# G-U-N/consolver

Hardware: AMD Instinct MI355X
Metric: images/sec at 8-step ConsistencySolver 512x512 (final latents; SD1.5 UNet fp16 + PPOScheduler, CFG 3) (higher is better)
Workload: dtype f16

## Files before the change

consolver_amd/csrc/attention.hip:

```cpp
#include "ops.h"
#include "el.h"
#include <type_traits>


namespace {

struct AttnParams {
    const f16* q; const f16* k; const f16* v; f16* out;
    int q_stride, k_stride, v_stride, out_stride;
    int H, Nq, Nk;
    float c;
    const float* bias;
    int nqb, lin0;
    int splits, tiles_per_split, part_rows;
    float* part_o;
    float* part_ml;
    int prio;
};

typedef __fp16 hf4 __attribute__((__vector_size__(4 * sizeof(__fp16))));
typedef __attribute__((address_space(3))) hf4* lds_hf4_ptr;

__device__ __forceinline__ u32x2 tr_read(const char* lds_addr) {
    hf4 r = __builtin_amdgcn_ds_read_tr16_b64_v4f16((lds_hf4_ptr)lds_addr);
// ... 758 lines not shown
                    for (int t = 0; t < 4; ++t) {
                        const u32x4 f = {pack2<f16>(s2[2 * t2][t][0], s2[2 * t2][t][1]), pack2<f16>(s2[2 * t2][t][2], s2[2 * t2][t][3]),
                                         pack2<f16>(s2[2 * t2 + 1][t][0], s2[2 * t2 + 1][t][1]), pack2<f16>(s2[2 * t2 + 1][t][2], s2[2 * t2 + 1][t][3])};
                        o_acc[a][t] = El<f16>::mfma(as_frag<f16>(vv.v), as_frag<f16>(f), o_acc[a][t]);
                    }
                }
            }
        }
#pragma unroll
        for (int t = 0; t < 4; ++t) lsum[t] = __shfl(o_acc[2][t][0], 32 + i16, 64);
    }
#pragma unroll
    for (int t = 0; t < 4; ++t) {
        const float inv = 1.0f / lsum[t];
        const int qrow = q0 + t * 16 + i16;
        f16* orow = p.out + (size_t)(b * p.Nq + qrow) * p.out_stride + h * DH;
#pragma unroll
        for (int a = 0; a < 3; ++a) {
            const int d = a * 16 + 4 * g;
            if (d + 4 <= DH) {
                const u32x2 o = {pack2<f16>(o_acc[a][t][0] * inv, o_acc[a][t][1] * inv), pack2<f16>(o_acc[a][t][2] * inv, o_acc[a][t][3] * inv)};
                *reinterpret_cast<u32x2*>(orow + d) = o;
            }
        }
    }
    if (TRACE && w == 0 && lane == 0 && blockIdx.x < A40_TRACE_SLOTS) {
        unsigned long long* tr = g_a40_trace + blockIdx.x * A40_TRACE_W;
        const unsigned long long te4 = __builtin_amdgcn_s_memrealtime();
        tr[5] = te1 - te0; tr[6] = tr0 - te1; tr[7] = te4 - te3; tr[8] = te0; tr[9] = te4;
        tr[10] = ((unsigned long long)__builtin_amdgcn_s_getreg((4 - 1) << 11 | 0 << 6 | 20) << 32) | __builtin_amdgcn_s_getreg((32 - 1) << 11 | 0 << 6 | 4);
    }
}

constexpr int ATTN_SLOTS = 512;

template <typename T, int DH, int QT, bool CAUSAL = false, bool BIAS = false>
int launch_attn(AttnParams p, int B, hipStream_t s, void* split_ws = nullptr, size_t split_ws_bytes = 0) {
    constexpr int DK = (DH + 31) / 32 * 32, DVP = (DH + 15) / 16 * 16;
    constexpr int KS = (DK == 64) ? 128 : ((DK * 2) % 64 == 32 ? DK * 2 : DK * 2 + 32);
    constexpr int VS = ((DVP * 2) % 64 == 32) ? DVP * 2 : DVP * 2 + 32;
    constexpr size_t lds = 2 * 64 * (size_t)(KS + VS);
    auto kfn = attn_kernel<T, DH, QT, CAUSAL, BIAS>;
    static bool configured = false;
    if (!configured) {
        CS_CHECK_HIP(hipFuncSetAttribute(reinterpret_cast<const void*>(kfn), hipFuncAttributeMaxDynamicSharedMemorySize, (int)lds));
        configured = true;
    }
    constexpr int ROWS = 4 * QT * 16;
    p.nqb = (p.Nq + ROWS - 1) / ROWS; p.lin0 = 0; p.splits = 1; p.tiles_per_split = 0; p.part_rows = 0; p.part_o = nullptr; p.part_ml = nullptr;
    const long total = (long)p.nqb * p.H * B;
    if (total > 0x7fffffffL) CS_FAIL(CS_E_SHAPE, "attention: too many workgroups");
    long main_wgs = total;
    if constexpr (DH == 128 && !CAUSAL && !BIAS) {
        const long tail = total % ATTN_SLOTS;
        const int tiles = (p.Nk + 63) / 64;
        if (split_ws && total > ATTN_SLOTS && tail > 0 && tail * 2 <= ATTN_SLOTS && tiles >= 8) {
            int splits = (int)std::min<long>(std::min<long>(ATTN_SLOTS / tail, 8), tiles / 4);
            const int per = (tiles + splits - 1) / splits;
            splits = (tiles + per - 1) / per;
            const size_t rows = (size_t)tail * ROWS;
            const size_t need = (size_t)splits * rows * (DH + 2) * sizeof(float);
            if (splits >= 2 && need <= split_ws_bytes) {
                main_wgs = total - tail;
                hipLaunchKernelGGL(kfn, dim3((unsigned)main_wgs), dim3(256), lds, s, p);
                AttnParams t = p;
                t.lin0 = (int)main_wgs; t.splits = splits; t.tiles_per_split = per; t.part_rows = (int)rows;
// ... 9 lines not shown
                CS_CHECK_LAUNCH();
                return CS_OK;
            }
        }
    }
    hipLaunchKernelGGL(kfn, dim3((unsigned)main_wgs), dim3(256), lds, s, p);
    CS_CHECK_LAUNCH();
    return CS_OK;
}

constexpr int A40_NS = 6;
int launch_attn40_lw(AttnParams p, int B, hipStream_t s) {
    constexpr size_t lds = (size_t)A40_NS * 12288;
    const bool trace = (tune().debug & 16384) != 0;
    auto kfn = trace ? ((tune().debug & 1) ? attn40_lw_kernel<A40_NS, true, 1> : (tune().debug & 2) ? attn40_lw_kernel<A40_NS, true, 2> : attn40_lw_kernel<A40_NS, true>)
                     : tune().attn_lw == 2 ? attn40_lw_kernel<A40_NS, false, 0, 0, false> : attn40_lw_kernel<A40_NS, false>;
    static bool configured = false;
    if (!configured) {
        CS_CHECK_HIP(hipFuncSetAttribute(reinterpret_cast<const void*>(attn40_lw_kernel<A40_NS, false>), hipFuncAttributeMaxDynamicSharedMemorySize, (int)lds));
        CS_CHECK_HIP(hipFuncSetAttribute(reinterpret_cast<const void*>(attn40_lw_kernel<A40_NS, false, 0, 0, false>), hipFuncAttributeMaxDynamicSharedMemorySize, (int)lds));
        CS_CHECK_HIP(hipFuncSetAttribute(reinterpret_cast<const void*>(attn40_lw_kernel<A40_NS, true>), hipFuncAttributeMaxDynamicSharedMemorySize, (int)lds));
        CS_CHECK_HIP(hipFuncSetAttribute(reinterpret_cast<const void*>(attn40_lw_kernel<A40_NS, true, 1>), hipFuncAttributeMaxDynamicSharedMemorySize, (int)lds));
        CS_CHECK_HIP(hipFuncSetAttribute(reinterpret_cast<const void*>(attn40_lw_kernel<A40_NS, true, 2>), hipFuncAttributeMaxDynamicSharedMemorySize, (int)lds));
        configured = true;
    }
    p.nqb = p.Nq / 256; p.lin0 = 0; p.splits = 1; p.tiles_per_split = 0; p.part_rows = 0; p.part_o = nullptr; p.part_ml = nullptr;
    const long total = (long)p.nqb * p.H * B;
    if (total > 0x7fffffffL) CS_FAIL(CS_E_SHAPE, "attention: too many workgroups");
    hipLaunchKernelGGL(kfn, dim3((unsigned)total), dim3(512), lds, s, p);
    CS_CHECK_LAUNCH();
    return CS_OK;
}

}

int debug_attn_trace_read(void* dst, size_t bytes) {
    if (bytes > sizeof(unsigned long long) * A40_TRACE_SLOTS * A40_TRACE_W) bytes = sizeof(unsigned long long) * A40_TRACE_SLOTS * A40_TRACE_W;
    return hipMemcpyFromSymbol(dst, HIP_SYMBOL(g_a40_trace), bytes, 0, hipMemcpyDeviceToHost) == hipSuccess ? CS_OK : CS_E_HIP;
}

size_t attention_split_workspace_bytes(int B, int H, int Nq, int Nk, int dh) {
    if (dh != 128) return 0;
    const long total = (long)((Nq + 127) / 128) * H * B, tail = total % ATTN_SLOTS;
    if (total <= ATTN_SLOTS || tail == 0 || tail * 2 > ATTN_SLOTS || (Nk + 63) / 64 < 8) return 0;
    return (size_t)8 * tail * 128 * (dh + 2) * sizeof(float);
}

int launch_attention(const AttnArgs& a, hipStream_t s) {
    if (!a.q || !a.k || !a.v || !a.out) CS_FAIL(CS_E_ARG, "attention: null pointer");
    if (a.B <= 0 || a.Nq <= 0) return a.B < 0 ? CS_E_SHAPE : CS_OK;
    if (a.Nk <= 0) CS_FAIL(CS_E_SHAPE, "attention: Nk must be positive");
    if ((a.q_stride | a.k_stride | a.v_stride | a.out_stride) & 7) CS_FAIL(CS_E_SHAPE, "attention: strides must be multiples of 8 halfs");
    AttnParams p;
    p.q = a.q; p.k = a.k; p.v = a.v; p.out = a.out;
    p.q_stride = a.q_stride; p.k_stride = a.k_stride; p.v_stride = a.v_stride; p.out_stride = a.out_stride;
    p.H = a.H; p.Nq = a.Nq; p.Nk = a.Nk;
    p.c = a.scale * 1.4426950408889634f;
    p.bias = a.bias;
    p.prio = tune().attn_prio < 0 ? (a.dh == 128 ? 1 : 0) : tune().attn_prio;
    if (a.bias) {
        if (a.dh != 64 || a.causal || a.Nk % 4) CS_FAIL(CS_E_UNSUPPORTED, "attention: the biased form is built for head dim 64, no mask, Nk %% 4 == 0");
        if (a.dtype == CS_BF16) return launch_attn<bf16_el, 64, 2, false, true>(p, a.B, s);
        return launch_attn<f16, 64, 2, false, true>(p, a.B, s);
    }
    if (a.causal) {
        if (a.dh != 64 || a.dtype == CS_BF16 || a.Nq != a.Nk) CS_FAIL(CS_E_UNSUPPORTED, "attention: the causal form is built for f16, head dim 64, Nq == Nk");
        return launch_attn<f16, 64, 2, true>(p, a.B, s);
    }
    switch (a.dh) {
        case 40: {
            const int qt = tune().attn_qt40;
            if (a.dtype == CS_BF16) CS_FAIL(CS_E_UNSUPPORTED, "attention: bf16 is built for head dim 128 only");
            if (tune().attn_lw && qt == 4 && a.Nq % 256 == 0 && a.Nk % 64 == 0) return launch_attn40_lw(p, a.B, s);
            if (qt == 4) return launch_attn<f16, 40, 4>(p, a.B, s);
            return launch_attn<f16, 40, 2>(p, a.B, s);
        }
        case 80: if (a.dtype == CS_BF16) break; return launch_attn<f16, 80, 2>(p, a.B, s);
        case 160: if (a.dtype == CS_BF16) break; return launch_attn<f16, 160, 1>(p, a.B, s);
        case 128:
            if (a.dtype == CS_BF16) return launch_attn<bf16_el, 128, 2>(p, a.B, s, a.split_ws, a.split_ws_bytes);
            return launch_attn<f16, 128, 2>(p, a.B, s, a.split_ws, a.split_ws_bytes);
        default: break;
    }
    CS_FAIL(CS_E_UNSUPPORTED, "attention: head dim %d / dtype %d not built (f16: 40/80/160/128, bf16: 128)", a.dh, a.dtype);
}
```

consolver_amd/csrc/ops.h:

```cpp
#pragma once
#include "common.h"

struct TuneSet {
    int halo = 1;
    int conv_lw = 1;
    int gemm_w8 = 1;
    int gemm_lw = 1;
    int gemm2_w8 = 1;
    int attn_lw = 1;
    int debug = 0;
    int gemm_gm = -1;
    int gn_fuse = 1;
    int cfg_share = 1;
    int xattn_fused = 1;
    int attn_prio = -1;
    int gemm2_prio = 0;
    int biggemm = 1;
    int attn_qt40 = 4;
    int x2_split_a = 1;
    int x2_sc_skip = 0;
    int ln_fold = 1;
    int xcd_grid = 1;
    int epi_fast = 3;
    int lo8 = 1;
    int conv_in_mfma = 1;
    int up_fold = 1;
    int head_x2 = 1;
    int conv_out_mfma = 1;
    int xattn_tile = 64;
};
extern TuneSet g_tune;
extern thread_local const TuneSet* t_tune;
inline const TuneSet& tune() { return t_tune ? *t_tune : g_tune; }
struct TuneScope {
    const TuneSet* prev;
    explicit TuneScope(const TuneSet* t) : prev(t_tune) { t_tune = t; }
    ~TuneScope() { t_tune = prev; }
    TuneScope(const TuneScope&) = delete; TuneScope& operator=(const TuneScope&) = delete;
};
int tune_apply(TuneSet& set, const char* key, int value);
TuneSet tune_snapshot();

// ... 131 lines not shown
```

consolver_amd/csrc/ops_api.cpp:

```cpp
#include "ops.h"
#include "../../include/consolver_hip_ops.h"
#include <cstring>

int debug_trace_read(void* dst, size_t bytes);
int debug_attn_trace_read(void* dst, size_t bytes);

#include <mutex>
TuneSet g_tune;
thread_local const TuneSet* t_tune = nullptr;
static std::mutex g_tune_write_mutex;

struct TuneKnob { const char* key; int TuneSet::* var; int lo, hi; bool pair; };
static const TuneKnob* tune_knobs(int* n) {
    static const TuneKnob k[] = {
        {"conv_halo", &TuneSet::halo, 0, 4, false},     {"gemm_lw", &TuneSet::gemm_lw, 0, 1, false},      {"gemm2_w8", &TuneSet::gemm2_w8, 0, 1, false},
        {"attn_lw", &TuneSet::attn_lw, 0, 2, false},    {"gemm_w8", &TuneSet::gemm_w8, 0, 1, false},      {"conv_lw", &TuneSet::conv_lw, 0, 3, false},
        {"gemm_big", &TuneSet::biggemm, 0, 3, false},   {"debug", &TuneSet::debug, 0, 0x7fffffff, false}, {"gemm_gm", &TuneSet::gemm_gm, -1, 64, false},
        {"gn_fuse", &TuneSet::gn_fuse, 0, 1, false},    {"xattn_fused", &TuneSet::xattn_fused, 0, 1, false}, {"cfg_share", &TuneSet::cfg_share, 0, 1, false},
        {"gemm2_prio", &TuneSet::gemm2_prio, -1, 1, false}, {"attn_prio", &TuneSet::attn_prio, -1, 1, false}, {"attn_qt40", &TuneSet::attn_qt40, 2, 4, true},
        {"x2_split_a", &TuneSet::x2_split_a, 0, 3, false}, {"x2_sc_skip", &TuneSet::x2_sc_skip, 0, 0xffff, false}, {"ln_fold", &TuneSet::ln_fold, 0, 1, false}, {"xcd_grid", &TuneSet::xcd_grid, 0, 1, false}, {"epi_fast", &TuneSet::epi_fast, 0, 3, false}, {"lo8", &TuneSet::lo8, 0, 1, false},
        {"conv_in_mfma", &TuneSet::conv_in_mfma, 0, 1, false}, {"xattn_tile", &TuneSet::xattn_tile, 64, 128, true},
        {"conv_out_mfma", &TuneSet::conv_out_mfma, 0, 1, false},
        {"up_fold", &TuneSet::up_fold, 0, 2, false},
        {"head_x2", &TuneSet::head_x2, 0, 1, false},
    };
    *n = (int)(sizeof(k) / sizeof(k[0]));
    return k;
}

int tune_apply(TuneSet& set, const char* key, int value) {
    if (!key) CS_FAIL(CS_E_ARG, "key is NULL");
    int n; const TuneKnob* k = tune_knobs(&n);
    for (int i = 0; i < n; ++i)
        if (!strcmp(key, k[i].key)) {
            const bool ok = k[i].pair ? (value == k[i].lo || value == k[i].hi) : (value >= k[i].lo && value <= k[i].hi);
            if (!ok) CS_FAIL(CS_E_ARG, "tuning key '%s': value %d outside %s%d%s%d%s", key, value, k[i].pair ? "{" : "[", k[i].lo, k[i].pair ? ", " : " .. ", k[i].hi, k[i].pair ? "}" : "]");
            set.*(k[i].var) = value;
            return CS_OK;
        }
    CS_FAIL(CS_E_ARG, "unknown tuning key '%s'", key);
}

TuneSet tune_snapshot() {
    std::lock_guard<std::mutex> lock(g_tune_write_mutex);
    return g_tune;
}

extern "C" {

int cs_set_tuning(const char* key, int value) {
    std::lock_guard<std::mutex> lock(g_tune_write_mutex);
    return tune_apply(g_tune, key, value);
}

int cs_get_tuning(const char* key, int* value) {
    if (!key || !value) CS_FAIL(CS_E_ARG, "key / value is NULL");
    int n; const TuneKnob* k = tune_knobs(&n);
// ... 321 lines not shown
```

consolver_amd/csrc/igemm.hip:

```cpp
#include "ops.h"
#include <stdlib.h>
#include <type_traits>


namespace {

constexpr int BM = 128;
constexpr int BK = 64;

__device__ __attribute__((aligned(256))) unsigned g_zero_page[64];

struct IgemmParams {
    const f16* a0; const f16* a1; int c0, c1;
    int Hi, Wi, Ho, Wo, HoWo;
    int stride, upsample;
    int pad_lo;
    int M, N, KT, cpt;
    int Ktot;
    const f16* w; const f16* bias; const f16* temb; int temb_stride; const f16* res; f16* out;
    const f16* res_lo; f16* out_lo;
    const f16* a0_lo; const f16* a1_lo; int KTh;
    float* row_stats;
    const float* ln_stats; int ln_groups; float ln_inv_c, ln_eps; const float* ln_s; const float* ln_b;
    int tiles_n, nblk;
// ... 1063 lines not shown
        g_trace[blockIdx.x * CS_TRACE_W + 5] = (unsigned long long)nsteps;
        g_trace[blockIdx.x * CS_TRACE_W + 0] = tw_entry;
        g_trace[blockIdx.x * CS_TRACE_W + 1] = tc_r0;
        g_trace[blockIdx.x * CS_TRACE_W + 2] = __builtin_amdgcn_s_memrealtime();
        g_trace[blockIdx.x * CS_TRACE_W + 4] = ((unsigned long long)__builtin_amdgcn_s_getreg((4 - 1) << 11 | 0 << 6 | 20) << 32) | __builtin_amdgcn_s_getreg((32 - 1) << 11 | 0 << 6 | 4);
    }
    __builtin_amdgcn_s_barrier();
    if (btab) __builtin_amdgcn_s_barrier();
    if constexpr (SUB) {
        const SubRows rows{wm * 64, b0, y0, x0, p.B, p.Ho, p.Wo, p.tw_shift, p.trw_shift, phase >> 1, phase & 1, phase * ((p.Ho * p.Wo) >> 8)};
        igemm_epilogue<false, NT, MT, NT, SubRows, 2, 0, true>(p.e, acc, rows, n_blk, lane, smem + w * 11264, btab ? smem + 4 * 11264 : nullptr);
        return;
    }
    const PatchRows rows{wm * 64, b0, y0, x0, p.B, p.Ho, p.Wo, p.tw_shift, p.trw_shift};
    if (p.splits == 1) {
        igemm_epilogue<false, NT, MT, NT, PatchRows, 2, 0, true>(p.e, acc, rows, n_blk, lane, smem + w * 11264, btab ? smem + 4 * 11264 : nullptr);
    } else {
        float* dst = p.partial + (size_t)blockIdx.y * p.e.M * p.e.N;
#pragma unroll
        for (int j = 0; j < MT; ++j) {
            const int m = rows(j * 16 + (lane & 15));
            if (m < 0) continue;
#pragma unroll
            for (int i = 0; i < NT; ++i)
                *reinterpret_cast<f32x4*>(dst + (size_t)m * p.e.N + n_blk + i * 16 + gq * 4) = acc[i][j];
        }
    }
    if (TRACE && w == 0 && lane == 0 && blockIdx.x < CS_TRACE_SLOTS && blockIdx.y == 0) {
        asm volatile("s_waitcnt vmcnt(0)" ::: "memory");
        g_trace[blockIdx.x * CS_TRACE_W + 3] = __builtin_amdgcn_s_memrealtime();
    }
}

template <int LNM = 0, int EPI = 0>
__global__ __launch_bounds__(512, 2) void gemm_lw_kernel(IgemmParams p) {
    constexpr int BMX = 256, BN = 160, NT = BN / 16, MT = 4, NWB = 3;
    constexpr int A_BYTES = BMX * 128, B_BYTES = BN * 128, STAGE = A_BYTES + B_BYTES;
    constexpr int APL = BMX / 8 / 4, WPL = BN / 8 / 4;
    extern __shared__ __attribute__((aligned(16))) char smem[];

    const int tid = threadIdx.x, lane = tid & 63;
    const int w = __builtin_amdgcn_readfirstlane(tid >> 6);
    int tm, tn;
    tile_of(blockIdx.x, p.nblk, p.tiles_n, p.gm, p.pn, tm, tn);
    const int m_blk = tm * BMX, n_blk = tn * BN;
    const int KT = p.KT;
    char* const lnx = smem + NWB * STAGE;

    if (w >= 4) {
        const int l = w - 4;

        const int pch = lane & 7, lr = lane >> 3;
        const f16* asrc0[APL]; const f16* asrc1[APL]; const f16* wsrc[WPL];
#pragma unroll
        for (int j = 0; j < APL; ++j) {
            const int r = 8 * (l + 4 * j) + lr;
            const long m = min(m_blk + r, p.M - 1);
            const int ch = (pch ^ ((r >> 1) & 7)) * 8;
            asrc0[j] = p.a0 + m * p.c0 + ch;
            asrc1[j] = p.c1 ? p.a1 + m * p.c1 + ch : asrc0[j];
        }
#pragma unroll
        for (int j = 0; j < WPL; ++j) {
            const int r = 8 * (l + 4 * j) + lr;
            wsrc[j] = p.w + (size_t)(n_blk + r) * p.Ktot + (pch ^ ((r >> 1) & 7)) * 8;
        }
// ... 660 lines not shown
constexpr size_t LN_LDS_W8 = 256 * 8 + 2 * 2 * 160 * 4, LN_LDS_LW = 256 * 8 + 2 * 160 * 4;

static int choose_xcd_grid(int tiles_m, int tiles_n, double a_bytes, double w_bytes) {
    if (!tune().xcd_grid) return 0;
    int best = 0; double best_cost = 0.85 * (a_bytes + 8.0 * w_bytes);
    for (int pn = 2; pn <= 8; pn *= 2) {
        const int px = 8 / pn;
        if (tiles_n % pn || tiles_m % px) continue;
        const double cost = pn * a_bytes + px * w_bytes;
        if (cost < best_cost) { best_cost = cost; best = pn; }
    }
    return best;
}

double igemm_flops(const IgemmArgs& a) {
    const double M = (double)a.B * a.Ho * a.Wo;
    return 2.0 * M * a.N * (double)a.taps * (a.c0 + a.c1);
}

template <bool UP, int BN, int KH, int SCHED>
static int launch_halo_sched(const HaloParams& h, dim3 grid, size_t lds, hipStream_t s) {
    static bool configured = false;
    if (!configured) {
        constexpr size_t max_lds = 2 * (HALO_ROWS_MAX * 128) + 3 * (160 * 128);
        CS_CHECK_HIP(hipFuncSetAttribute(reinterpret_cast<const void*>(conv3_halo_kernel<UP, BN, KH, SCHED>), hipFuncAttributeMaxDynamicSharedMemorySize, (int)max_lds));
        configured = true;
    }
    hipLaunchKernelGGL((conv3_halo_kernel<UP, BN, KH, SCHED>), grid, dim3(512), lds, s, h);
    CS_CHECK_LAUNCH();
    return CS_OK;
}
template <bool UP, int BN, int KH>
static int launch_halo(const HaloParams& h, dim3 grid, size_t lds, hipStream_t s) { return launch_halo_sched<UP, BN, KH, KH == 2 ? 2 : 0>(h, grid, lds, s); }

struct LaunchInfo { bool gn_done = false; int row_groups = 0; };
static int launch_igemm_impl(const IgemmArgs& a, hipStream_t s, LaunchInfo* li) {
    const int cin = a.c0 + a.c1;
    if (!a.a0 || !a.w || !a.out) CS_FAIL(CS_E_ARG, "igemm: a0, w, out required");
    if (a.taps != 1 && a.taps != 9) CS_FAIL(CS_E_ARG, "igemm: taps must be 1 or 9");
    if (cin % BK || a.c0 % BK || (a.c1 && !a.a1)) CS_FAIL(CS_E_SHAPE, "igemm: channels (%d,%d) must be multiples of %d", a.c0, a.c1, BK);
    if (a.B <= 0 || a.Ho <= 0 || a.Wo <= 0) return (a.B < 0) ? CS_E_SHAPE : CS_OK;
    if (a.taps == 1 && (a.stride != 1 || a.upsample || a.Hi != a.Ho || a.Wi != a.Wo)) CS_FAIL(CS_E_ARG, "igemm: 1x1 needs stride 1, no upsample");
    if (a.geglu && (a.N % 256) && (a.N % 320)) CS_FAIL(CS_E_SHAPE, "igemm: GEGLU needs N %% 256 == 0 or N %% 320 == 0 (N=%d)", a.N);
    IgemmParams p;
    p.a0 = a.a0; p.a1 = a.a1; p.c0 = a.c0; p.c1 = a.c1;
    p.Hi = a.Hi; p.Wi = a.Wi; p.Ho = a.Ho; p.Wo = a.Wo; p.HoWo = a.Ho * a.Wo;
    p.stride = a.stride; p.upsample = a.upsample; p.pad_lo = a.pad_after_only ? 0 : 1;
    if (a.pad_after_only && !(a.taps == 9 && a.stride == 2)) CS_FAIL(CS_E_ARG, "igemm: pad_after_only is the stride-2 3x3 form");
    p.M = a.B * a.Ho * a.Wo; p.N = a.N; p.cpt = cin / BK; p.KT = a.taps * p.cpt; p.Ktot = a.taps * cin;
    p.w = a.w; p.bias = a.bias; p.temb = a.temb; p.temb_stride = a.temb_stride; p.res = a.res; p.out = a.out;
    p.res_lo = a.res ? a.res_lo : nullptr; p.out_lo = a.out_lo; p.lo8 = (a.lo8 && (p.res_lo || p.out_lo)) ? 1 : 0;
    const bool conv3_early = a.taps == 9;
    p.row_stats = a.row_stats;
    p.ln_stats = a.ln_stats; p.ln_groups = a.ln_groups; p.ln_inv_c = 1.0f / (float)cin; p.ln_eps = a.ln_eps; p.ln_s = a.ln_s; p.ln_b = a.ln_b;
    if (a.ln_stats) {
        if (a.taps != 1 || a.c1 || a.temb || a.res || a.out_lo || a.row_stats || a.gn_stats)
            CS_FAIL(CS_E_ARG, "igemm: a folded LayerNorm (ln_stats) is the epilogue of a plain linear layer (one source, no temb / residual / lo plane / statistics)");
        if (!a.ln_s || !a.ln_b || a.ln_groups < 1) CS_FAIL(CS_E_ARG, "igemm: ln_stats needs ln_s, ln_b and ln_groups >= 1");
    }
    if (a.row_stats && (a.geglu || a.gn_stats)) CS_FAIL(CS_E_ARG, "igemm: row_stats excludes GEGLU and gn_stats");
    if (a.row_stats && !a.row_stats_groups) CS_FAIL(CS_E_ARG, "igemm: row_stats needs row_stats_groups (the layout the chosen kernel wrote is returned there)");
    p.a0_lo = a.a0_lo; p.a1_lo = a.c1 ? a.a1_lo : nullptr; p.KTh = p.KT;
    const int lnm = a.ln_stats ? 1 : (a.row_stats && !conv3_early ? 2 : 0);
    const bool split_a = a.a0_lo != nullptr;
    if (split_a) {
        if (a.taps != 1 || a.geglu) CS_FAIL(CS_E_ARG, "igemm: a split-fp16 A operand (a0_lo) is built for 1x1 / linear layers without GEGLU");
// ... 69 lines not shown
        }
        const bool pays = tiles_m * tiles_n * splits >= 160;
        const int tin_w = a.upsample ? TW / 2 : TW, tin_h = a.upsample ? TH / 2 : TH;
        HaloParams h;
        h.HALO_W = tin_w + 2; h.HALO_IMG = (tin_h + 2) * (tin_w + 2); h.NHALO = IPT * h.HALO_IMG; h.NQ = (h.NHALO + 7) / 8;
        if ((pays || use_halo == 2 || use_halo == 3) && h.NHALO <= HALO_ROWS_MAX && h.NQ <= 64 && (PP == 1 || IPT == 1)) {
            h.e = p; h.e.tiles_n = tiles_n; h.e.nblk = tiles_m * tiles_n; h.e.row_stats = nullptr; h.e.pn = choose_xcd_grid(tiles_m, tiles_n, a_bytes, w_bytes);
            h.x = a.a0; h.w = a.w; h.Cin = cin; h.H = a.Hi; h.W = a.Wi; h.B = a.B; h.NC = NC; h.Ho = Ho; h.Wo = Wo;
            h.tw_shift = TW == 16 ? 4 : 3; h.trw_shift = 0; while ((1 << h.trw_shift) < TRW) ++h.trw_shift;
            h.PX = PX; h.PP = PP;
            h.splits = splits; h.partial = a.splitk_ws; h.sched = wide ? 2 : 0;
            const size_t l = 2 * (HALO_ROWS_MAX * 128) + 3 * ((size_t)hbn * (wide ? 64 : 128));
            const dim3 grid(h.e.nblk, splits);
            int rc;
            if (lw) {
                constexpr size_t llw_max = 2 * (HALO_ROWS_MAX * 128) + 3 * (160 * 128);
                const size_t llw = 2 * ((size_t)h.NQ * 1024) + 3 * ((size_t)hbn * 128);
                const bool fast = TW == 16 && TH == 16 && tune().conv_lw != 2 && (a.upsample ? (h.HALO_W == 10 && h.NQ == 13) : (h.HALO_W == 18 && h.NQ == 41));
                const bool fast8 = hbn == 160 && TW == 8 && TH == 8 && !a.upsample && IPT == 4 && PP == 1 && h.HALO_W == 10 && h.NQ == 50 && tune().conv_lw != 2 &&
                                   !((tune().debug & 16384) != 0);
                typedef void (*lw_fn)(HaloParams);
                static const lw_fn variants[11] = {conv3_lw_kernel<false, 160, false, true>, conv3_lw_kernel<false, 160>, conv3_lw_kernel<true, 160>,
                                                   conv3_lw_kernel<false, 160, true, true>, conv3_lw_kernel<false, 160, true, false>, conv3_lw_kernel<true, 160, false, true>,
                                                   conv3_lw_kernel<false, 128, false, true>, conv3_lw_kernel<false, 128>, conv3_lw_kernel<true, 128>, conv3_lw_kernel<true, 128, false, true>,
                                                   conv3_lw_kernel<false, 160, false, 2>};
                static bool configured_lw = false;
                if (!configured_lw) {
                    for (lw_fn f : variants)
                        CS_CHECK_HIP(hipFuncSetAttribute(reinterpret_cast<const void*>(f), hipFuncAttributeMaxDynamicSharedMemorySize, (int)llw_max));
                    configured_lw = true;
                }
                auto launch = [&](lw_fn kfn) -> int { hipLaunchKernelGGL(kfn, grid, dim3(512), llw, s, h); return CS_OK; };
                const bool trace = (tune().debug & 16384) && !a.upsample;
                if (fast8) rc = launch(variants[10]);
                else if (hbn == 128) rc = launch(variants[a.upsample ? (fast ? 9 : 8) : (fast ? 6 : 7)]);
                else if (trace) rc = launch(variants[fast ? 3 : 4]);
                else if (a.upsample) rc = launch(variants[fast ? 5 : 2]);
                else rc = launch(variants[fast ? 0 : 1]);
                if (rc != CS_OK) return rc;
                rc = CS_OK;
            } else if (wide && hbn == 320) rc = a.upsample ? launch_halo<true, 320, 2>(h, grid, l, s) : launch_halo<false, 320, 2>(h, grid, l, s);
            else if (wide) rc = a.upsample ? launch_halo<true, 256, 2>(h, grid, l, s) : launch_halo<false, 256, 2>(h, grid, l, s);
            else if (hbn == 160) rc = a.upsample ? launch_halo<true, 160, 1>(h, grid, l, s) : launch_halo<false, 160, 1>(h, grid, l, s);
            else rc = a.upsample ? launch_halo<true, 128, 1>(h, grid, l, s) : launch_halo<false, 128, 1>(h, grid, l, s);
            if (rc != CS_OK) return rc;
            CS_CHECK_LAUNCH();
            li->gn_done = stats_ok && (splits == 1 || reduce_leaves_stats(h.e));
            if (splits > 1) return launch_splitk_reduce(h.e, (const float*)a.splitk_ws, splits, s);
            return CS_OK;
        }
    }
    if (a.geglu && conv3) CS_FAIL(CS_E_ARG, "igemm: GEGLU epilogue only for linear layers");
    if (tune().biggemm && !conv3 && a.N % 320 == 0) {
        const int tiles_m = (p.M + 255) / 256, tn = a.N / 320;
        if (tiles_m * tn >= 192 || tune().biggemm == 2) {
            p.tiles_n = tn; p.nblk = tiles_m * tn; p.pn = choose_xcd_grid(tiles_m, tn, a_bytes, w_bytes); li->gn_done = stats_ok; li->row_groups = a.N / 160;
            p.gm = tune().gemm_gm >= 0 ? (tune().gemm_gm > 1 ? tune().gemm_gm : 1) : (tn >= 12 ? 4 : 1);
            constexpr size_t lds = 2 * (256 * BK * 2 + 320 * BK * 2);
            static bool configured = false;
            if (!configured) {
                CS_CHECK_HIP(hipFuncSetAttribute(reinterpret_cast<const void*>(gemm_big_kernel<false, 320>), hipFuncAttributeMaxDynamicSharedMemorySize, (int)lds));
                CS_CHECK_HIP(hipFuncSetAttribute(reinterpret_cast<const void*>(gemm_big_kernel<true, 320>), hipFuncAttributeMaxDynamicSharedMemorySize, (int)lds));
                configured = true;
            }
            const bool off32 = (double)p.M * (a.c0 > a.c1 ? a.c0 : a.c1) * 2 < 4.0e9 && (double)a.N * p.Ktot * 2 < 4.0e9;
            if ((split_a || lnm || epi == 1) && !(tune().gemm_w8 && off32 && !tune().debug)) goto generic_tiles;
            if (tune().gemm_w8 && off32 && !tune().debug) {
// ... 126 lines not shown
```

Baseline: 72.37.

## Add warp-specialized loader-wave attention kernel for head dims 80 and 160

Adds a new attention kernel in which four dedicated loader waves stream K/V tiles into an NS-deep LDS ring with async global-to-LDS copies, while the compute waves run MFMA softmax-attention. It also adds a lazy max-rescale step that skips the online-softmax rescale unless some lane's score exceeds the running max by a threshold. The kernel is enabled by default for SD1.5's head dims 80 and 160 (the mid and low resolution attention levels), replacing the generic kernel there. The aim is to hide K/V load latency behind compute, at the cost of extra waves per block and a large LDS footprint that may lower occupancy.

Result: no change. 72.85, median of 6 (+0.7%).

```diff
diff --git a/consolver_amd/csrc/attention.hip b/consolver_amd/csrc/attention.hip
--- a/consolver_amd/csrc/attention.hip
+++ b/consolver_amd/csrc/attention.hip
@@ -814,6 +814,219 @@
     }
 }
 
+template <int DH>
+struct AttnLwGeom {
+    static constexpr int RS = ((DH * 2) % 64 == 32) ? DH * 2 : DH * 2 + 32;
+    static constexpr int TB = 64 * RS, ST = 2 * TB;
+    static constexpr int NP = ST / 1024;
+    static_assert(TB % 1024 == 0, "a DMA piece must not straddle the K and V tiles");
+    static_assert(NP % 4 == 0, "pieces per loader wave");
+};
+
+template <int DH, int QT, int NCW, int NS>
+__global__ __launch_bounds__(64 * (NCW + 4)) void attn_lw_kernel(AttnParams p) {
+    typedef El<f16>::frag frag;
+    using G = AttnLwGeom<DH>;
+    constexpr int RS = G::RS, TB = G::TB, ST = G::ST, NP = G::NP, PW = NP / 4;
+    constexpr int DK = (DH + 31) / 32 * 32, KSTEPS = DK / 32, DVT = DH / 16, CPR = DH / 8;
+    static_assert(DH % 16 == 0, "no spare V column: the denominator is summed in registers");
+    static_assert(NS >= 3 && (size_t)NS * ST <= 160 * 1024, "ring depth / LDS");
+    static_assert(PW * (NS - 2) <= 63, "vmcnt range");
+    extern __shared__ __attribute__((aligned(16))) char smem[];
+    const int tid = threadIdx.x, lane = tid & 63;
+    const int w = __builtin_amdgcn_readfirstlane(tid >> 6);
+    const int g = lane >> 4, i16 = lane & 15;
+    int lin;
+    {
+        const int n = gridDim.x, bid = blockIdx.x, xcd = bid & 7, q = n >> 3, r = n & 7;
+        lin = (xcd < r ? xcd * (q + 1) : r * (q + 1) + (xcd - r) * q) + (bid >> 3);
+    }
+    const int qblk = lin % p.nqb, hb = lin / p.nqb;
+    const int h = hb % p.H, b = hb / p.H;
+    const int ntiles = p.Nk >> 6;
+
+    if (w >= NCW) {
+        const int l = w - NCW;
+        const char* src[PW]; size_t step[PW];
+#pragma unroll
+        for (int j = 0; j < PW; ++j) {
+            const int off = (l + 4 * j) * 1024 + lane * 16, kv = off >= TB ? 1 : 0, o2 = off - kv * TB;
+            const int row = o2 / RS, ch = (o2 - row * RS) >> 4;
+            const int stride = kv ? p.v_stride : p.k_stride;
+            const f16* base = (kv ? p.v : p.k) + (size_t)b * p.Nk * stride + h * DH;
+            if (ch < CPR) { src[j] = reinterpret_cast<const char*>(base + (size_t)row * stride + ch * 8); step[j] = (size_t)64 * stride * 2; }
+            else { src[j] = reinterpret_cast<const char*>(g_attn_ones_chunk + 4); step[j] = 0; }
+        }
+        auto issue = [&](int tile, int stage) {
+            const int t = tile < ntiles ? tile : ntiles - 1;
+#pragma unroll
+            for (int j = 0; j < PW; ++j) glds16a(src[j] + (size_t)t * step[j], smem + stage * ST + (l + 4 * j) * 1024);
+        };
+        for (int t = 0; t < NS - 1; ++t) issue(t, t);
+        int st = NS - 1;
+        for (int j = 0; j < ntiles; ++j) {
+            asm volatile("s_waitcnt vmcnt(%0)" :: "n"(PW * (NS - 2)) : "memory");
+            __builtin_amdgcn_s_barrier();
+            issue(j - 1 + NS, st);
+            st = st + 1 == NS ? 0 : st + 1;
+        }
+        asm volatile("s_waitcnt vmcnt(0)" ::: "memory");
+        return;
+    }
+
+    const int q0 = qblk * (NCW * QT * 16) + w * (QT * 16);
+    frag qf[QT][KSTEPS];
+    {
+        u32x4 raw[QT][KSTEPS];
+#pragma unroll
+        for (int t = 0; t < QT; ++t) {
+            const int qrow = q0 + t * 16 + i16;
+#pragma unroll
+            for (int ks = 0; ks < KSTEPS; ++ks) {
+                const int d = ks * 32 + 8 * g, dc = d < DH ? d : 0;
+                raw[t][ks] = *reinterpret_cast<const u32x4*>(p.q + ((size_t)(b * p.Nq + qrow) * p.q_stride + h * DH + dc));
+            }
+        }
+#pragma unroll
+        for (int t = 0; t < QT; ++t) {
+#pragma unroll
+            for (int ks = 0; ks < KSTEPS; ++ks) {
+                const bool ok = ks * 32 + 8 * g < DH;
+                u32x4 v = raw[t][ks];
+#pragma unroll
+                for (int e = 0; e < 4; ++e)
+                    v[e] = ok ? pack2<f16>(El<f16>::tof((u16)(v[e] & 0xffff)) * p.c, El<f16>::tof((u16)(v[e] >> 16)) * p.c) : 0u;
+                qf[t][ks] = as_frag<f16>(v);
+            }
+        }
+    }
+    f32x4 o_acc[DVT][QT];
+#pragma unroll
+    for (int a = 0; a < DVT; ++a)
+#pragma unroll
+        for (int t = 0; t < QT; ++t) o_acc[a][t] = f32x4{0.f, 0.f, 0.f, 0.f};
+    float m_run[QT], l_run[QT];
+#pragma unroll
+    for (int t = 0; t < QT; ++t) { m_run[t] = 0.f; l_run[t] = 0.f; }
+
+    constexpr float THR = 8.0f;
+    auto do_tile = [&](const char* tk, auto first_tag) {
+        constexpr bool FIRST = decltype(first_tag)::value;
+        const char* tv = tk + TB;
+        f32x4 s[4][QT];
+        f32x4 negm[QT];
+#pragma unroll
+        for (int t = 0; t < QT; ++t) { const float v = FIRST ? 0.f : -m_run[t]; negm[t] = f32x4{v, v, v, v}; }
+        {
+            constexpr int NF = 4 * KSTEPS, RING = 4;
+            auto kaddr = [&](int f) {
+                const int kt = f / KSTEPS, ks = f - kt * KSTEPS;
+                return tk + (kt * 16 + i16) * RS + (ks * 32 + 8 * g) * 2;
+            };
+            frag kf[RING];
+#pragma unroll
+            for (int f = 0; f < RING; ++f) kf[f] = *reinterpret_cast<const frag*>(kaddr(f));
+            __builtin_amdgcn_sched_barrier(0);
+#pragma unroll
+            for (int f = 0; f < NF; ++f) {
+                const int kt = f / KSTEPS, ks = f - kt * KSTEPS;
+#pragma unroll
+                for (int t = 0; t < QT; ++t)
+                    s[kt][t] = El<f16>::mfma(kf[f % RING], qf[t][ks], ks == 0 ? negm[t] : s[kt][t]);
+                if (f + RING < NF) kf[f % RING] = *reinterpret_cast<const frag*>(kaddr(f + RING));
+                __builtin_amdgcn_sched_barrier(0);
+            }
+        }
+        float mxl[QT];
+        bool over = false;
+#pragma unroll
+        for (int t = 0; t < QT; ++t) {
+            float mx = s[0][t][0];
+#pragma unroll
+            for (int kt = 0; kt < 4; ++kt)
+#pragma unroll
+                for (int r = 0; r < 4; ++r) mx = fmaxf(mx, s[kt][t][r]);
+            mxl[t] = mx;
+            over |= mx > THR;
+        }
+        if (FIRST || __builtin_amdgcn_ballot_w64(over) != 0) {
+#pragma unroll
+            for (int t = 0; t < QT; ++t) {
+                const float mx = xor32_max(xor16_max(mxl[t]));
+                const float delta = FIRST ? mx : fmaxf(mx, 0.f);
+                m_run[t] = FIRST ? delta : m_run[t] + delta;
+                if (!FIRST) {
+                    const float alpha = __builtin_amdgcn_exp2f(-delta);
+                    l_run[t] *= alpha;
+#pragma unroll
+                    for (int a = 0; a < DVT; ++a) o_acc[a][t] *= alpha;
+                }
+#pragma unroll
+                for (int kt = 0; kt < 4; ++kt)
+#pragma unroll
+                    for (int r = 0; r < 4; ++r) s[kt][t][r] -= delta;
+            }
+        }
+        frag pf[QT][2];
+#pragma unroll
+        for (int t = 0; t < QT; ++t) {
+            float ps = 0.f;
+#pragma unroll
+            for (int kt = 0; kt < 4; ++kt)
+#pragma unroll
+                for (int r = 0; r < 4; ++r) {
+                    const float e = __builtin_amdgcn_exp2f(s[kt][t][r]);
+                    s[kt][t][r] = e;
+                    ps += e;
+                }
+            l_run[t] += ps;
+#pragma unroll
+            for (int t2 = 0; t2 < 2; ++t2) {
+                u32x4 f;
+                f[0] = pack2<f16>(s[2 * t2][t][0], s[2 * t2][t][1]); f[1] = pack2<f16>(s[2 * t2][t][2], s[2 * t2][t][3]);
+                f[2] = pack2<f16>(s[2 * t2 + 1][t][0], s[2 * t2 + 1][t][1]); f[3] = pack2<f16>(s[2 * t2 + 1][t][2], s[2 * t2 + 1][t][3]);
+                pf[t][t2] = as_frag<f16>(f);
+            }
+        }
+#pragma unroll
+        for (int t2 = 0; t2 < 2; ++t2) {
+#pragma unroll
+            for (int a = 0; a < DVT; ++a) {
+                const char* addr = tv + (32 * t2 + 4 * g + (i16 >> 2)) * RS + (a * 16 + 4 * (i16 & 3)) * 2;
+                const u32x2 lo = tr_read(addr);
+                const u32x2 hi = tr_read(addr + 16 * RS);
+                const frag vf = as_frag<f16>(u32x4{lo[0], lo[1], hi[0], hi[1]});
+#pragma unroll
+                for (int t = 0; t < QT; ++t) o_acc[a][t] = El<f16>::mfma(vf, pf[t][t2], o_acc[a][t]);
+            }
+        }
+    };
+    __syncthreads();
+    do_tile(smem, std::true_type{});
+    int so = 0;
+    for (int j = 1; j < ntiles; ++j) {
+        so = so + ST == NS * ST ? 0 : so + ST;
+        __syncthreads();
+        do_tile(smem + so, std::false_type{});
+    }
+
+#pragma unroll
+    for (int t = 0; t < QT; ++t) {
+        float l = l_run[t];
+        l += __shfl_xor(l, 16, 64);
+        l += __shfl_xor(l, 32, 64);
+        const float inv = 1.0f / l;
+        const int qrow = q0 + t * 16 + i16;
+        f16* orow = p.out + (size_t)(b * p.Nq + qrow) * p.out_stride + h * DH;
+#pragma unroll
+        for (int a = 0; a < DVT; ++a) {
+            const int d = a * 16 + 4 * g;
+            const u32x2 o = {pack2<f16>(o_acc[a][t][0] * inv, o_acc[a][t][1] * inv), pack2<f16>(o_acc[a][t][2] * inv, o_acc[a][t][3] * inv)};
+            *reinterpret_cast<u32x2*>(orow + d) = o;
+        }
+    }
+}
+
 constexpr int ATTN_SLOTS = 512;
 
 template <typename T, int DH, int QT, bool CAUSAL = false, bool BIAS = false>
@@ -889,6 +1102,23 @@
     return CS_OK;
 }
 
+template <int DH, int QT, int NCW, int NS>
+int launch_attn_lw(AttnParams p, int B, hipStream_t s) {
+    constexpr size_t lds = (size_t)NS * AttnLwGeom<DH>::ST;
+    auto kfn = attn_lw_kernel<DH, QT, NCW, NS>;
+    static bool configured = false;
+    if (!configured) {
+        CS_CHECK_HIP(hipFuncSetAttribute(reinterpret_cast<const void*>(kfn), hipFuncAttributeMaxDynamicSharedMemorySize, (int)lds));
+        configured = true;
+    }
+    p.nqb = p.Nq / (NCW * QT * 16); p.lin0 = 0; p.splits = 1; p.tiles_per_split = 0; p.part_rows = 0; p.part_o = nullptr; p.part_ml = nullptr;
+    const long total = (long)p.nqb * p.H * B;
+    if (total > 0x7fffffffL) CS_FAIL(CS_E_SHAPE, "attention: too many workgroups");
+    hipLaunchKernelGGL(kfn, dim3((unsigned)total), dim3(64 * (NCW + 4)), lds, s, p);
+    CS_CHECK_LAUNCH();
+    return CS_OK;
+}
+
 }
 
 int debug_attn_trace_read(void* dst, size_t bytes) {
@@ -932,8 +1162,20 @@
             if (qt == 4) return launch_attn<f16, 40, 4>(p, a.B, s);
             return launch_attn<f16, 40, 2>(p, a.B, s);
         }
-        case 80: if (a.dtype == CS_BF16) break; return launch_attn<f16, 80, 2>(p, a.B, s);
-        case 160: if (a.dtype == CS_BF16) break; return launch_attn<f16, 160, 1>(p, a.B, s);
+        case 80: {
+            if (a.dtype == CS_BF16) break;
+            const int lw = tune().attn_lw_wide;
+            if (lw == 1 && a.Nq % 256 == 0 && a.Nk % 64 == 0) return launch_attn_lw<80, 2, 8, 6>(p, a.B, s);
+            if (lw == 2 && a.Nq % 128 == 0 && a.Nk % 64 == 0) return launch_attn_lw<80, 2, 4, 6>(p, a.B, s);
+            return launch_attn<f16, 80, 2>(p, a.B, s);
+        }
+        case 160: {
+            if (a.dtype == CS_BF16) break;
+            const int lw = tune().attn_lw_wide;
+            if (lw == 1 && a.Nq % 128 == 0 && a.Nk % 64 == 0) return launch_attn_lw<160, 1, 8, 3>(p, a.B, s);
+            if (lw == 2 && a.Nq % 64 == 0 && a.Nk % 64 == 0) return launch_attn_lw<160, 1, 4, 3>(p, a.B, s);
+            return launch_attn<f16, 160, 1>(p, a.B, s);
+        }
         case 128:
             if (a.dtype == CS_BF16) return launch_attn<bf16_el, 128, 2>(p, a.B, s, a.split_ws, a.split_ws_bytes);
             return launch_attn<f16, 128, 2>(p, a.B, s, a.split_ws, a.split_ws_bytes);
diff --git a/consolver_amd/csrc/ops.h b/consolver_amd/csrc/ops.h
--- a/consolver_amd/csrc/ops.h
+++ b/consolver_amd/csrc/ops.h
@@ -8,6 +8,7 @@
     int gemm_lw = 1;
     int gemm2_w8 = 1;
     int attn_lw = 1;
+    int attn_lw_wide = 1;
     int debug = 0;
     int gemm_gm = -1;
     int gn_fuse = 1;
diff --git a/consolver_amd/csrc/ops_api.cpp b/consolver_amd/csrc/ops_api.cpp
--- a/consolver_amd/csrc/ops_api.cpp
+++ b/consolver_amd/csrc/ops_api.cpp
@@ -14,7 +14,7 @@
 static const TuneKnob* tune_knobs(int* n) {
     static const TuneKnob k[] = {
         {"conv_halo", &TuneSet::halo, 0, 4, false},     {"gemm_lw", &TuneSet::gemm_lw, 0, 1, false},      {"gemm2_w8", &TuneSet::gemm2_w8, 0, 1, false},
-        {"attn_lw", &TuneSet::attn_lw, 0, 2, false},    {"gemm_w8", &TuneSet::gemm_w8, 0, 1, false},      {"conv_lw", &TuneSet::conv_lw, 0, 3, false},
+        {"attn_lw", &TuneSet::attn_lw, 0, 2, false},    {"attn_lw_wide", &TuneSet::attn_lw_wide, 0, 2, false},    {"gemm_w8", &TuneSet::gemm_w8, 0, 1, false},      {"conv_lw", &TuneSet::conv_lw, 0, 3, false},
         {"gemm_big", &TuneSet::biggemm, 0, 3, false},   {"debug", &TuneSet::debug, 0, 0x7fffffff, false}, {"gemm_gm", &TuneSet::gemm_gm, -1, 64, false},
         {"gn_fuse", &TuneSet::gn_fuse, 0, 1, false},    {"xattn_fused", &TuneSet::xattn_fused, 0, 1, false}, {"cfg_share", &TuneSet::cfg_share, 0, 1, false},
         {"gemm2_prio", &TuneSet::gemm2_prio, -1, 1, false}, {"attn_prio", &TuneSet::attn_prio, -1, 1, false}, {"attn_qt40", &TuneSet::attn_qt40, 2, 4, true},
```

## Add persistent 3x3 conv kernel that prefetches next tile across tile boundaries

Applied to the files above, without the earlier changes.

Adds a persistent variant of the warp-specialized halo 3x3 conv kernel. It launches at most 256 blocks, and each block loops over tiles with a stride of the grid size. Loader waves start fetching the next tile's halo and weights while the current tile's last channel chunk is still computing, and the MFMA waves alternate the halo buffer parity between tiles. The aim is to hide the per-tile prologue and fill latency and the block launch tail on large non-upsample convs. The cost is a larger, more complex kernel with extra barriers, and possible load imbalance. It is enabled by default through a new conv_persist tune knob.

New measurement: 72.85 before, 72.81 after. About the same (-0.0%).

```diff
diff --git a/consolver_amd/csrc/igemm.hip b/consolver_amd/csrc/igemm.hip
--- a/consolver_amd/csrc/igemm.hip
+++ b/consolver_amd/csrc/igemm.hip
@@ -1119,6 +1119,229 @@
     }
 }
 
+template <int BN>
+__global__ __launch_bounds__(512, 2) void conv3_lw_persist_kernel(HaloParams p) {
+    constexpr int TAPS = 9, TL = TAPS - 1;
+    constexpr int NT = BN / 16, MT = 4;
+    constexpr int A_BYTES = 41 * 1024, B_BYTES = BN * 128, NWB = 3;
+    constexpr int NBQ = BN / 8, WPL = NBQ / 4;
+    static_assert(NBQ % 4 == 0, "every loader wave issues the same number of weight pieces");
+    constexpr int PATCH = 11264, TAIL = 2 * A_BYTES + NWB * B_BYTES, NP = 2 * B_BYTES / PATCH < 3 ? 2 * B_BYTES / PATCH : 3;
+    constexpr int BIAS_TAB = TAIL + (4 - NP) * PATCH;
+    static_assert(NP == (BN == 160 ? 3 : 2) && BIAS_TAB + BN * 2 <= 160 * 1024, "epilogue patches");
+    extern __shared__ __attribute__((aligned(16))) char smem[];
+    char* const lA = smem;
+    char* const lB = smem + 2 * A_BYTES;
+
+    const int tid = threadIdx.x, lane = tid & 63;
+    const int w = __builtin_amdgcn_readfirstlane(tid >> 6);
+    const int G = gridDim.x, NC = p.NC, nblk = p.e.nblk;
+    const bool btab = p.e.bias != nullptr;
+    struct Tile { int n_blk, b0, y0, x0; };
+    auto tile_at = [&](int t) {
+        Tile r;
+        int tm, tn;
+        int nb = nblk, tiles_n = p.e.tiles_n, pn = p.e.pn, PP = p.PP, PX = p.PX;
+        asm volatile("" : "+s"(nb), "+s"(tiles_n), "+s"(pn), "+s"(PP), "+s"(PX));
+        tile_of(t, nb, tiles_n, 1, pn, tm, tn);
+        r.n_blk = tn * BN;
+        if (PP == 1) { r.b0 = tm << (8 - p.trw_shift); r.y0 = 0; r.x0 = 0; }
+        else {
+            r.b0 = tm / PP;
+            const int pr = tm - r.b0 * PP, py = pr / PX, px = pr - py * PX;
+            r.y0 = py << (p.trw_shift - p.tw_shift); r.x0 = px << p.tw_shift;
+        }
+        return r;
+    };
+    int t = blockIdx.x;
+
+    if (w >= 4) {
+        const int l = w - 4;
+        const int pch = lane & 7;
+        const float inv_img = 1.0f / (float)p.HALO_IMG, inv_w = 1.0f / (float)p.HALO_W;
+        const char* zero = reinterpret_cast<const char*>(g_zero_region) + pch * 16;
+        auto halo_src = [&](const Tile& T, int k, int lr) -> const char* {
+            const int q = (k & 7) * 4 + l + (k >> 3) * 32;
+            const int hr = 8 * q + lr;
+            const int hi = (int)(((float)hr + 0.5f) * inv_img), rem = hr - hi * p.HALO_IMG;
+            const int hy = (int)(((float)rem + 0.5f) * inv_w), hx = rem - hy * p.HALO_W;
+            const int b = T.b0 + hi, y = T.y0 - 1 + hy, x = T.x0 - 1 + hx;
+            const bool ok = (q < p.NQ) & (hr < p.NHALO) & (b < p.B) & (y >= 0) & (y < p.H) & (x >= 0) & (x < p.W);
+            const long pix = ((long)b * p.H + y) * p.W + x;
+            return ok ? reinterpret_cast<const char*>(p.x + pix * p.Cin + (pch ^ (hx & 7)) * 8) : zero;
+        };
+        auto w_src = [&](const Tile& T, int j, int lr) -> const f16* {
+            const int q = l + 4 * j, r = 8 * (q < NBQ ? q : 0) + lr;
+            return p.w + (size_t)(T.n_blk + r) * (TAPS * p.Cin) + (pch ^ ((r >> 1) & 7)) * 8;
+        };
+        Tile cur = tile_at(t);
+        const char* hsrc[16]; const char* hnext[16];
+        const f16* wsrc[WPL]; const f16* wnext[WPL];
+#pragma unroll
+        for (int k = 0; k < 16; ++k) { hsrc[k] = halo_src(cur, k, lane >> 3); hnext[k] = hsrc[k]; }
+#pragma unroll
+        for (int j = 0; j < WPL; ++j) { wsrc[j] = w_src(cur, j, lane >> 3); wnext[j] = wsrc[j]; }
+        auto issue_w = [&](const auto& ws, int c, int tap, int buf) {
+            const size_t koff = (size_t)tap * p.Cin + c * BK;
+#pragma unroll
+            for (int j = 0; j < WPL; ++j) glds16(ws[j] + koff, lB + buf * B_BYTES + (l + 4 * j) * 1024);
+        };
+        auto issue_h = [&](const auto& hs, int c, auto s_tag, int buf) -> int {
+            constexpr int S = decltype(s_tag)::value;
+            const int q0 = S * 4 + l, q1 = q0 + 32;
+            int n = 0;
+            if (q0 < p.NQ) { glds16(hs[S] + (size_t)c * 128, lA + buf * A_BYTES + q0 * 1024); ++n; }
+            if (q1 < p.NQ) { glds16(hs[S + 8] + (size_t)c * 128, lA + buf * A_BYTES + q1 * 1024); ++n; }
+            return n;
+        };
+        static_for<8>([&](auto sc) { issue_h(hsrc, 0, sc, 0); });
+        issue_w(wsrc, 0, 0, 0);
+        asm volatile("s_waitcnt vmcnt(0)" ::: "memory");
+        __builtin_amdgcn_s_barrier();
+        int ab = 0, wb1 = 1;
+        for (;;) {
+            const bool more = t + G < nblk;
+            const Tile nxt = tile_at(more ? t + G : t);
+            int lr_t = lane >> 3;
+            asm volatile("" : "+v"(lr_t));
+            f16x8 bias_reg = {0, 0, 0, 0, 0, 0, 0, 0};
+            if (btab && l == 0 && lane < BN / 8) bias_reg = *reinterpret_cast<const f16x8*>(p.e.bias + cur.n_blk + lane * 8);
+            for (int c = 0; c < NC; ++c) {
+                const int abn = ab ^ 1;
+                const bool cross = c + 1 == NC;
+                const bool halo_next = !cross || more;
+                auto halo_slice = [&](auto s_tag) -> int {
+                    constexpr int S = decltype(s_tag)::value;
+                    if (c == 0) { hnext[S] = halo_src(nxt, S, lr_t); hnext[S + 8] = halo_src(nxt, S + 8, lr_t); }
+                    if (!halo_next) return 0;
+                    return cross ? issue_h(hnext, 0, s_tag, abn) : issue_h(hsrc, c + 1, s_tag, abn);
+                };
+                auto step = [&](auto t_tag) {
+                    constexpr int T = decltype(t_tag)::value;
+                    const bool last = T == TL && !halo_next;
+                    if constexpr (T == TL) {
+                        if (c == 0) {
+#pragma unroll
+                            for (int j = 0; j < WPL; ++j) wnext[j] = w_src(nxt, j, lr_t);
+                        }
+                        if (!last) { if (cross) issue_w(wnext, 0, 0, wb1); else issue_w(wsrc, c + 1, 0, wb1); }
+                    } else issue_w(wsrc, c, T + 1, wb1);
+                    int nh = 0;
+                    if constexpr (T < 8) nh = halo_slice(std::integral_constant<int, T>{});
+                    if (nh == 0) asm volatile("s_waitcnt vmcnt(0)" ::: "memory");
+                    else if (nh == 1) asm volatile("s_waitcnt vmcnt(1)" ::: "memory");
+                    else asm volatile("s_waitcnt vmcnt(2)" ::: "memory");
+                    __builtin_amdgcn_s_barrier();
+                    wb1 = wb1 == NWB - 1 ? 0 : wb1 + 1;
+                };
+                static_for<TAPS>(step);
+                ab = abn;
+            }
+            __builtin_amdgcn_s_barrier();
+            if (btab) {
+                if (l == 0 && lane < BN / 8) *reinterpret_cast<f16x8*>(smem + BIAS_TAB + lane * 16) = bias_reg;
+                asm volatile("s_waitcnt lgkmcnt(0)" ::: "memory");
+                __builtin_amdgcn_s_barrier();
+            }
+            if (!more) return;
+            t += G; cur = nxt;
+#pragma unroll
+            for (int k = 0; k < 16; ++k) hsrc[k] = hnext[k];
+#pragma unroll
+            for (int j = 0; j < WPL; ++j) wsrc[j] = wnext[j];
+            __builtin_amdgcn_s_barrier();
+        }
+    }
+
+    const int wm = w;
+    const unsigned lA_base = lds_addr(lA), lB_base = lds_addr(lB);
+    constexpr int NQ = 2 * NT, RS = NT / 2, LA = RS - 1, QB = NQ - LA;
+    static_assert(NT % 2 == 0 && NQ % RS == 0 && LA >= 2 && MT == 4 && QB + 1 < NQ && QB > NT + MT, "ring / fragment placement");
+    static_assert(LA == 3 || LA == 4, "prologue reads");
+    constexpr int HW_F = 18, ROWB = HW_F * 128;
+    int par = 0;
+    for (;;) {
+        const Tile cur = tile_at(t);
+        int lane_t = lane;
+        asm volatile("" : "+v"(lane_t));
+        const int gq = lane_t >> 4, swz = (lane_t >> 1) & 7, fxl = lane_t & 15;
+        const unsigned wfrag0 = (lane_t & 15) * 128 + (gq ^ swz) * 16, wfrag1 = (lane_t & 15) * 128 + ((4 + gq) ^ swz) * 16;
+        f32x4 acc[NT][MT];
+#pragma unroll
+        for (int i = 0; i < NT; ++i)
+#pragma unroll
+            for (int j = 0; j < MT; ++j) acc[i][j] = f32x4{0.f, 0.f, 0.f, 0.f};
+        f16x8 fa[2][MT], fw[RS];
+        const unsigned rowb = lA_base + (unsigned)(par * A_BYTES) + (unsigned)(4 * wm * HW_F) * 128;
+        unsigned VA[3][2], VN, WB[NWB][2];
+#pragma unroll
+        for (int d = 0; d < 3; ++d) {
+            const int hcol = fxl + d;
+            const unsigned sw = (unsigned)((gq ^ (hcol & 7)) << 4);
+            VA[d][0] = rowb + hcol * 128 + sw; VA[d][1] = rowb + hcol * 128 + (sw ^ 64u);
+        }
+#pragma unroll
+        for (int b3 = 0; b3 < NWB; ++b3) { WB[b3][0] = lB_base + b3 * B_BYTES + wfrag0; WB[b3][1] = lB_base + b3 * B_BYTES + wfrag1; }
+        int delta = par ? -A_BYTES : A_BYTES;
+        VN = VA[0][0] + delta;
+        __builtin_amdgcn_s_barrier();
+        lds_read<0>(fw[0], WB[0][0]); lds_read<lw_rowf(1, false, 0, 0) * ROWB>(fa[0][0], VA[0][0]); lds_read<lw_rowf(1, false, 1, 0) * ROWB>(fa[0][1], VA[0][0]);
+        lds_read<2048>(fw[1], WB[0][0]); lds_read<lw_rowf(1, false, 2, 0) * ROWB>(fa[0][2], VA[0][0]); lds_read<lw_rowf(1, false, 3, 0) * ROWB>(fa[0][3], VA[0][0]);
+        lds_read<2 * 2048>(fw[2], WB[0][0]);
+        if constexpr (LA == 4) lds_read<3 * 2048>(fw[3], WB[0][0]);
+        for (int c = 0; c < NC; ++c) {
+            static_for<TAPS>([&](auto tc) {
+                constexpr int T = decltype(tc)::value;
+                constexpr int TN = T == TL ? 0 : T + 1;
+                constexpr int DY = T / 3, DX = T % 3, DYN = TN / 3, DXN = TN % 3;
+                constexpr int WBC = T % 3, WBN = (T + 1) % 3;
+                static_for<NQ>([&](auto qc) {
+                    constexpr int q = decltype(qc)::value, ks = q / NT, i = q - ks * NT;
+                    if constexpr (q == QB) __builtin_amdgcn_s_barrier();
+                    {
+                        constexpr int r = q + LA;
+                        if constexpr (r < NT) lds_read<r * 2048>(fw[r % RS], WB[WBC][0]);
+                        else if constexpr (r < NQ) lds_read<(r - NT) * 2048>(fw[r % RS], WB[WBC][1]);
+                        else lds_read<(r - NQ) * 2048>(fw[r % RS], WB[WBN][0]);
+                    }
+                    if constexpr (q < MT) lds_read<lw_rowf(1, false, q, DY) * ROWB>(fa[1][q], VA[DX][1]);
+                    if constexpr (q == QB || q == QB + 1) {
+                        constexpr int j0 = (q - QB) * 2;
+                        if constexpr (T == TL) {
+                            lds_read<lw_rowf(1, false, j0, 0) * ROWB>(fa[0][j0], VN); lds_read<lw_rowf(1, false, j0 + 1, 0) * ROWB>(fa[0][j0 + 1], VN);
+                        } else {
+                            lds_read<lw_rowf(1, false, j0, DYN) * ROWB>(fa[0][j0], VA[DXN][0]); lds_read<lw_rowf(1, false, j0 + 1, DYN) * ROWB>(fa[0][j0 + 1], VA[DXN][0]);
+                        }
+                    }
+                    asm volatile("s_waitcnt lgkmcnt(%0)" :: "n"(lw_wait_count(q, NQ, LA, MT, QB)));
+                    __builtin_amdgcn_sched_barrier(0);
+#pragma unroll
+                    for (int j = 0; j < MT; ++j) mfma_inplace(acc[i][j], fw[q % RS], fa[ks][j]);
+                    __builtin_amdgcn_sched_barrier(0);
+                });
+            });
+#pragma unroll
+            for (int d = 0; d < 3; ++d) { VA[d][0] += delta; VA[d][1] += delta; }
+            VN -= delta; delta = -delta;
+        }
+        asm volatile("s_waitcnt lgkmcnt(0)\n s_nop 7\n s_nop 7" ::: "memory");
+#pragma unroll
+        for (int i = 0; i < NT; ++i)
+#pragma unroll
+            for (int j = 0; j < MT; ++j) asm volatile("" : "+v"(acc[i][j]));
+        __builtin_amdgcn_s_barrier();
+        if (btab) __builtin_amdgcn_s_barrier();
+        char* const patch = wm < NP ? lB + B_BYTES + wm * PATCH : smem + TAIL + (wm - NP) * PATCH;
+        char* const btable = btab ? smem + BIAS_TAB : nullptr;
+        const PatchRows rows{wm * 64, cur.b0, cur.y0, cur.x0, p.B, p.Ho, p.Wo, p.tw_shift, p.trw_shift};
+        igemm_epilogue<false, NT, MT, NT, PatchRows, 2, 0, true>(p.e, acc, rows, cur.n_blk, lane_t, patch, btable);
+        t += G;
+        if (t >= nblk) return;
+        par ^= NC & 1;
+        asm volatile("s_waitcnt lgkmcnt(0)" ::: "memory");
+    }
+}
+
 template <int LNM = 0, int EPI = 0>
 __global__ __launch_bounds__(512, 2) void gemm_lw_kernel(IgemmParams p) {
     constexpr int BMX = 256, BN = 160, NT = BN / 16, MT = 4, NWB = 3;
@@ -1845,6 +2068,21 @@
 }
 template <bool UP, int BN, int KH>
 static int launch_halo(const HaloParams& h, dim3 grid, size_t lds, hipStream_t s) { return launch_halo_sched<UP, BN, KH, KH == 2 ? 2 : 0>(h, grid, lds, s); }
+
+constexpr int LW_PERSIST_GRID = 256;
+static int launch_lw_persist(const HaloParams& h, int bn, hipStream_t s) {
+    typedef void (*lw_fn)(HaloParams);
+    static const lw_fn k[2] = {conv3_lw_persist_kernel<160>, conv3_lw_persist_kernel<128>};
+    static bool configured = false;
+    if (!configured) {
+        for (lw_fn f : k) CS_CHECK_HIP(hipFuncSetAttribute(reinterpret_cast<const void*>(f), hipFuncAttributeMaxDynamicSharedMemorySize, 160 * 1024));
+        configured = true;
+    }
+    const size_t lds = 2 * 41 * 1024 + 3 * ((size_t)bn * 128) + (bn == 160 ? 1 : 2) * 11264 + bn * 2;
+    hipLaunchKernelGGL(k[bn == 128 ? 1 : 0], dim3(h.e.nblk < LW_PERSIST_GRID ? h.e.nblk : LW_PERSIST_GRID, 1), dim3(512), lds, s, h);
+    CS_CHECK_LAUNCH();
+    return CS_OK;
+}
 
 struct LaunchInfo { bool gn_done = false; int row_groups = 0; };
 static int launch_igemm_impl(const IgemmArgs& a, hipStream_t s, LaunchInfo* li) {
@@ -1980,7 +2218,8 @@
                 }
                 auto launch = [&](lw_fn kfn) -> int { hipLaunchKernelGGL(kfn, grid, dim3(512), llw, s, h); return CS_OK; };
                 const bool trace = (tune().debug & 16384) && !a.upsample;
-                if (fast8) rc = launch(variants[10]);
+                if (fast && !a.upsample && splits == 1 && !trace && tune().conv_persist && h.e.nblk > LW_PERSIST_GRID) rc = launch_lw_persist(h, hbn, s);
+                else if (fast8) rc = launch(variants[10]);
                 else if (hbn == 128) rc = launch(variants[a.upsample ? (fast ? 9 : 8) : (fast ? 6 : 7)]);
                 else if (trace) rc = launch(variants[fast ? 3 : 4]);
                 else if (a.upsample) rc = launch(variants[fast ? 5 : 2]);
diff --git a/consolver_amd/csrc/ops.h b/consolver_amd/csrc/ops.h
--- a/consolver_amd/csrc/ops.h
+++ b/consolver_amd/csrc/ops.h
@@ -4,6 +4,7 @@
 struct TuneSet {
     int halo = 1;
     int conv_lw = 1;
+    int conv_persist = 1;
     int gemm_w8 = 1;
     int gemm_lw = 1;
     int gemm2_w8 = 1;
diff --git a/consolver_amd/csrc/ops_api.cpp b/consolver_amd/csrc/ops_api.cpp
--- a/consolver_amd/csrc/ops_api.cpp
+++ b/consolver_amd/csrc/ops_api.cpp
@@ -23,6 +23,7 @@
         {"conv_out_mfma", &TuneSet::conv_out_mfma, 0, 1, false},
         {"up_fold", &TuneSet::up_fold, 0, 2, false},
         {"head_x2", &TuneSet::head_x2, 0, 1, false},
+        {"conv_persist", &TuneSet::conv_persist, 0, 1, false},
     };
     *n = (int)(sizeof(k) / sizeof(k[0]));
     return k;
```
